# zhizdev/sparsefusion

Measured on AMD Instinct MI355X. Metric: novel views/sec, distillation steps (2 NGP renders fwd+bwd + VAE enc/dec + 51-eval PLMS + LPIPS), 256^2 / 32x32 latents, 2-view synthetic hydrant, higher is better.
Workload: dtype bf16 MFMA operands / f32 accumulate (UNet); f32 (NGP render)

## Files before the change

### include/sparsefusion_hip.h

```cpp
#ifndef SPARSEFUSION_HIP_H
#define SPARSEFUSION_HIP_H

#include <stdint.h>

#ifdef __cplusplus
extern "C" {
#endif

#define SF_OK 0
#define SF_ERR_INVALID 1
#define SF_ERR_LAUNCH 2

const char* sf_last_error(void);
int sf_abi_version(void);
int sf_operand_is_f16(void);


int sf_grid_encode_forward(const float* inputs, const float* embeddings,
                           const int32_t* offsets, float* outputs,
                           uint32_t B, uint32_t D, uint32_t C, uint32_t L,
                           float S, uint32_t H, float* dy_dx,
                           uint32_t gridtype, int align_corners,
                           const int32_t* h_offsets, void* stream);

// ... 82 lines not shown
  float* g_w2; float* g_b2;
} sf_ngp_field_grad;

int sf_ngp_density(const sf_ngp_field* f, const float* xyz, uint32_t P,
                   float* sigma, float* albedo, void* stream);


int sf_ngp_density_lattice(const sf_ngp_field* f, const float* ax, const float* ay, const float* az,
                           uint32_t nx, uint32_t ny, uint32_t nz, float* sigma, void* stream);

int sf_ngp_point_attrs(const sf_ngp_field* f, const float* xyz, uint32_t P, float epsilon,
                       float* sigma, float* albedo, float* grad, float* normal, void* stream);

int sf_ngp_texture_bake(const sf_ngp_field* f, const float* verts, uint32_t V, const int32_t* faces, uint32_t F, uint32_t W,
                        uint8_t* rgb8, float* albedo, float* xyz, int32_t* face_id, void* stream);

uint64_t sf_gaussian3d_workspace_bytes(uint32_t nx, uint32_t ny, uint32_t nz);
int sf_gaussian3d(const float* in, float* out, uint32_t nx, uint32_t ny, uint32_t nz,
                  float sigma, float truncate, double* stats, void* workspace,
                  uint64_t workspace_bytes, void* stream);

uint64_t sf_mc_workspace_bytes(uint32_t nx, uint32_t ny, uint32_t nz);
int sf_mc_count(const float* vol, uint32_t nx, uint32_t ny, uint32_t nz, float iso,
                void* workspace, uint64_t workspace_bytes, uint32_t* counts2, void* stream);
int sf_mc_emit(const float* vol, uint32_t nx, uint32_t ny, uint32_t nz, float iso,
               void* workspace, uint64_t workspace_bytes, float* verts, int32_t* faces,
               void* stream);

int sf_ngp_render_forward(const sf_ngp_field* f, const float* rays_o,
                          const float* rays_d, const float* aabb, uint32_t N,
                          uint32_t T, float min_near, const float* lin,
                          const float* u_coarse, const float* u_fine,
                          uint32_t u_fine_row_stride, float bg_color, float* nears,
                          float* fars, float* z_sorted, float* sigma_s,
                          float* rgb_s, float* image, float* depth,
                          float* weights_sum, float* field_cache, float* workspace,
                          uint64_t workspace_bytes, void* stream);

int sf_ngp_render_backward(const sf_ngp_field* f, const sf_ngp_field_grad* g,
                           const float* rays_o, const float* rays_d,
                           const float* aabb, uint32_t N, uint32_t T,
                           const float* nears, const float* fars,
                           const float* z_sorted, const float* sigma_s,
                           const float* rgb_s, float bg_color,
                           const float* grad_image, const float* grad_weights_sum,
                           uint32_t rays_per_row, const float* field_cache,
                           float* workspace, uint64_t workspace_bytes,
                           void* stream);

uint64_t sf_ngp_render_workspace_bytes(uint32_t N, uint32_t T);
uint64_t sf_ngp_render_forward_workspace_bytes(uint32_t N, uint32_t T);

uint64_t sf_ngp_render_cache_bytes(uint32_t N, uint32_t T);

int sf_ngp_render_shaded_forward(const sf_ngp_field* f, const float* rays_o, const float* rays_d, const float* aabb,
                                 uint32_t N, uint32_t T, float min_near, const float* lin, const float* u_coarse,
                                 const float* u_fine, uint32_t u_fine_row_stride, float bg_color, const float* light_d,
                                 float ambient_ratio, float epsilon, float* nears, float* fars, float* z_sorted,
                                 float* sigma_s, float* rgb_s, float* normal_s, float* rgb_shaded_s, float* xyz_s,
                                 float* image, float* normal_image, float* orient, float* depth, float* weights_sum,
                                 float* workspace, uint64_t workspace_bytes, void* stream);
uint64_t sf_ngp_render_shaded_workspace_bytes(uint32_t N, uint32_t T);

int sf_ngp_render_occ_eval(const sf_ngp_field* f, const float* rays_o, const float* rays_d,
                           const float* nears, const float* fars, const uint8_t* grid,
                           float dt_gamma, uint32_t max_steps, uint32_t C, uint32_t H,
                           const float* noises, float T_thresh, uint32_t N,
                           float* weights_sum, float* depth, float* image, void* stream);

int sf_ngp_render_occ_eval_shaded(const sf_ngp_field* f, const float* rays_o, const float* rays_d,
        const float* nears, const float* fars, const uint8_t* grid, float dt_gamma, uint32_t max_steps,
        uint32_t C, uint32_t H, const float* noises, float T_thresh, uint32_t N,
        const float* light_d , float ambient_ratio, float epsilon,
        float* weights_sum, float* depth, float* image,
        float* normal_image , uint32_t* n_samples ,
        void* stream);


enum {
  SF_OP_CONV = 1,
  SF_OP_GN_ACT = 2,
  SF_OP_LN = 3,
  SF_OP_GEMV = 4,
  SF_OP_ATTN = 5,
  SF_OP_GCA_POOL = 6,
  SF_OP_ELTWISE = 7,
  SF_OP_MEMSET = 8,
  SF_OP_TIME_EMB = 9,
  SF_OP_SPLITK_REDUCE = 10,
  SF_OP_POOL = 11,
  SF_OP_LPIPS = 12,
  SF_OP_EFT = 13,
  SF_OP_FCONV = 14,
  SF_OP_SLOTS = 15,
  SF_OP_GCA = 16,
  SF_OP_INITX = 17,
  SF_OP_GN_FINALIZE = 18
};

typedef struct {
  int32_t type;
  int32_t flags;
  void* p[24];
  int32_t i[32];
  float f[8];
} sf_op;
// ... 61 lines not shown
```

### sparsefusion_amd/_lib.py

```python
import ctypes as C
import os

import torch

_HERE = os.path.dirname(os.path.abspath(__file__))
_DEFAULT_LIB = "libsparsefusion_hip_f16.so" if os.environ.get("SF_OPERAND", "bf16").lower() in ("f16", "fp16", "half") else "libsparsefusion_hip.so"
LIB_PATH = os.environ.get("SF_HIP_LIB") or os.path.join(_HERE, _DEFAULT_LIB)

_lib = None

c_f32p = C.c_void_p
c_i32p = C.c_void_p
u32 = C.c_uint32
u64 = C.c_uint64


class SfNgpField(C.Structure):
    _fields_ = [("embeddings", C.c_void_p), ("h_offsets", C.c_void_p), ("L", u32), ("S", C.c_float),
                ("H", u32), ("gridtype", u32),
                ("w0", C.c_void_p), ("b0", C.c_void_p), ("w1", C.c_void_p), ("b1", C.c_void_p),
                ("w2", C.c_void_p), ("b2", C.c_void_p), ("bound", C.c_float)]


class SfNgpFieldGrad(C.Structure):
# ... 24 lines not shown
    "sf_last_error": (C.c_char_p, []),
    "sf_abi_version": (C.c_int, []),
    "sf_operand_is_f16": (C.c_int, []),
    "sf_grid_encode_forward": (C.c_int, [c_f32p, c_f32p, c_i32p, c_f32p, u32, u32, u32, u32, C.c_float, u32,
                                         c_f32p, u32, C.c_int, C.c_void_p, C.c_void_p]),
    "sf_grid_encode_backward": (C.c_int, [c_f32p, c_f32p, c_f32p, c_i32p, c_f32p, u32, u32, u32, u32, C.c_float,
                                          u32, c_f32p, c_f32p, u32, C.c_int, C.c_void_p, C.c_void_p]),
    "sf_near_far_from_aabb": (C.c_int, [c_f32p, c_f32p, c_f32p, u32, C.c_float, c_f32p, c_f32p, C.c_void_p]),
    "sf_morton3D": (C.c_int, [c_i32p, u32, c_i32p, C.c_void_p]),
    "sf_morton3D_invert": (C.c_int, [c_i32p, u32, c_i32p, C.c_void_p]),
    "sf_packbits": (C.c_int, [c_f32p, u32, C.c_float, C.c_void_p, C.c_void_p]),
    "sf_occ_mark_untrained": (C.c_int, [c_f32p, c_f32p, u32, C.c_float, u32, u32, c_f32p, c_i32p, C.c_void_p, C.c_void_p]),
    "sf_sph_from_ray": (C.c_int, [c_f32p, c_f32p, C.c_float, u32, c_f32p, C.c_void_p]),
    "sf_march_rays_train_workspace_bytes": (u64, [u32]),
    "sf_march_rays_train": (C.c_int, [c_f32p, c_f32p, C.c_void_p, C.c_float, C.c_float, u32, u32, u32, u32, u32, c_f32p,
                                      c_f32p, c_f32p, c_f32p, c_f32p, c_i32p, c_i32p, c_f32p, C.c_void_p, u64, C.c_void_p]),
    "sf_composite_rays_train_forward": (C.c_int, [c_f32p, c_f32p, c_f32p, c_i32p, u32, u32, C.c_float, c_f32p, c_f32p,
                                                  c_f32p, C.c_void_p]),
    "sf_composite_rays_train_backward": (C.c_int, [c_f32p, c_f32p, c_f32p, c_f32p, c_f32p, c_i32p, c_f32p, c_f32p, u32,
                                                   u32, C.c_float, c_f32p, c_f32p, C.c_void_p]),
    "sf_march_rays": (C.c_int, [u32, u32, c_i32p, c_f32p, c_f32p, c_f32p, C.c_float, C.c_float, u32, u32, u32,
                                C.c_void_p, c_f32p, c_f32p, c_f32p, c_f32p, c_f32p, c_f32p, C.c_void_p]),
    "sf_composite_rays": (C.c_int, [u32, u32, C.c_float, c_i32p, c_f32p, c_f32p, c_f32p, c_f32p, c_f32p, c_f32p,
                                    c_f32p, C.c_void_p]),
    "sf_adam_multi": (C.c_int, [C.POINTER(SfAdamArgs), C.c_void_p]),
    "sf_loss_partial_rows": (u32, []),
    "sf_upsample2x_forward": (C.c_int, [c_f32p, c_f32p, u32, u32, u32, C.c_void_p]),
    "sf_upsample2x_backward": (C.c_int, [c_f32p, c_f32p, u32, u32, u32, C.c_void_p]),
    "sf_render_loss_forward": (C.c_int, [c_f32p, c_f32p, c_f32p, c_f32p, u64, u64, C.c_float, c_f32p, C.c_void_p]),
    "sf_render_loss_backward": (C.c_int, [c_f32p, c_f32p, c_f32p, c_f32p, u64, u64, C.c_float, C.c_float, C.c_float, C.c_float,
                                          C.c_float, c_f32p, c_f32p, c_f32p, C.c_void_p]),
    "sf_fusion_loss_forward": (C.c_int, [c_f32p, c_f32p, c_f32p, c_f32p, u32, u64, u64, c_f32p, C.c_void_p]),
    "sf_fusion_loss_backward": (C.c_int, [c_f32p, c_f32p, c_f32p, c_f32p, u32, u64, u64, C.c_float, C.c_float, C.c_float,
                                          c_f32p, c_f32p, c_f32p, C.c_void_p]),
    "sf_ngp_density": (C.c_int, [C.POINTER(SfNgpField), c_f32p, u32, c_f32p, c_f32p, C.c_void_p]),
    "sf_ngp_density_lattice": (C.c_int, [C.POINTER(SfNgpField), c_f32p, c_f32p, c_f32p, u32, u32, u32, c_f32p, C.c_void_p]),
    "sf_ngp_point_attrs": (C.c_int, [C.POINTER(SfNgpField), c_f32p, u32, C.c_float, c_f32p, c_f32p, c_f32p, c_f32p, C.c_void_p]),
    "sf_ngp_texture_bake": (C.c_int, [C.POINTER(SfNgpField), c_f32p, u32, c_i32p, u32, u32, C.c_void_p, c_f32p, c_f32p, c_i32p,
                                      C.c_void_p]),
    "sf_gaussian3d_workspace_bytes": (u64, [u32, u32, u32]),
    "sf_gaussian3d": (C.c_int, [c_f32p, c_f32p, u32, u32, u32, C.c_float, C.c_float, C.c_void_p, C.c_void_p, u64, C.c_void_p]),
    "sf_mc_workspace_bytes": (u64, [u32, u32, u32]),
    "sf_mc_count": (C.c_int, [c_f32p, u32, u32, u32, C.c_float, C.c_void_p, u64, C.c_void_p, C.c_void_p]),
    "sf_mc_emit": (C.c_int, [c_f32p, u32, u32, u32, C.c_float, C.c_void_p, u64, c_f32p, c_i32p, C.c_void_p]),
    "sf_ngp_render_forward": (C.c_int, [C.POINTER(SfNgpField), c_f32p, c_f32p, c_f32p, u32, u32, C.c_float,
                                        c_f32p, c_f32p, c_f32p, u32, C.c_float, c_f32p, c_f32p, c_f32p, c_f32p,
                                        c_f32p, c_f32p, c_f32p, c_f32p, c_f32p, c_f32p, u64, C.c_void_p]),
    "sf_ngp_render_backward": (C.c_int, [C.POINTER(SfNgpField), C.POINTER(SfNgpFieldGrad), c_f32p, c_f32p,
                                         c_f32p, u32, u32, c_f32p, c_f32p, c_f32p, c_f32p, c_f32p,
                                         C.c_float, c_f32p, c_f32p, u32, c_f32p, c_f32p, u64, C.c_void_p]),
    "sf_ngp_render_workspace_bytes": (u64, [u32, u32]),
    "sf_ngp_render_forward_workspace_bytes": (u64, [u32, u32]),
    "sf_ngp_render_cache_bytes": (u64, [u32, u32]),
    "sf_ngp_render_shaded_forward": (C.c_int, [C.POINTER(SfNgpField), c_f32p, c_f32p, c_f32p, u32, u32, C.c_float, c_f32p, c_f32p,
                                               c_f32p, u32, C.c_float, c_f32p, C.c_float, C.c_float, c_f32p, c_f32p, c_f32p,
                                               c_f32p, c_f32p, c_f32p, c_f32p, c_f32p, c_f32p, c_f32p, c_f32p, c_f32p, c_f32p,
                                               c_f32p, u64, C.c_void_p]),
    "sf_ngp_render_shaded_workspace_bytes": (u64, [u32, u32]),
    "sf_ngp_render_occ_eval": (C.c_int, [C.POINTER(SfNgpField), c_f32p, c_f32p, c_f32p, c_f32p, C.c_void_p, C.c_float, u32, u32, u32,
                                         c_f32p, C.c_float, u32, c_f32p, c_f32p, c_f32p, C.c_void_p]),
    "sf_ngp_render_occ_eval_shaded": (C.c_int, [C.POINTER(SfNgpField), c_f32p, c_f32p, c_f32p, c_f32p, C.c_void_p, C.c_float, u32, u32,
                                                u32, c_f32p, C.c_float, u32, c_f32p, C.c_float, C.c_float, c_f32p, c_f32p, c_f32p,
                                                c_f32p, C.c_void_p, C.c_void_p]),
    "sf_plan_run": (C.c_int, [C.POINTER(SfOp), u32, C.c_void_p]),
    "sf_conv_igemm_t_launches": (u64, []),
    "sf_gca4_launches": (u64, [C.c_int]),
    "sf_plan_profile": (C.c_int, [C.POINTER(SfOp), u32, C.c_void_p, C.c_void_p]),
    "sf_conv_packed_elems": (u64, [u32, u32, u32, u32]),
    "sf_conv_pack_weights": (C.c_int, [C.c_void_p, u32, u32, u32, u32, u32, C.c_void_p]),
    "sf_plms_update": (C.c_int, [c_f32p, c_f32p, c_f32p, C.c_void_p, u64, c_f32p, c_f32p, C.c_void_p]),
    "sf_plms_combine": (C.c_int, [c_f32p, c_f32p, c_f32p, c_f32p, C.c_void_p, u64, c_f32p, c_f32p, C.c_void_p]),
    "sf_plms_step": (C.c_int, [c_f32p, c_f32p, c_f32p, c_f32p, C.c_void_p, c_f32p, c_f32p, c_f32p, C.c_void_p, u64, c_f32p, c_f32p, c_f32p, u64, C.c_void_p]),
}


_handles = {}


def _load(path):
    if path not in _handles:
        if not os.path.exists(path):
            raise RuntimeError(
                f"{path} is missing: build it with `python -m sparsefusion_amd.build` (`--f16` for the IEEE-half operand build; "
                "there is no CPU fallback for the sparsefusion_amd hot path)")
        handle = C.CDLL(path)
        for name, (res, args) in SIGNATURES.items():
            fn = getattr(handle, name)
            fn.restype = res
            fn.argtypes = args
        _handles[path] = handle
    return _handles[path]


def lib(operand=None):
    global _lib
    if operand is None:
        if _lib is None:
            _lib = _load(LIB_PATH)
        return _lib
    if operand == "f16":
        return _load(os.path.join(_HERE, "libsparsefusion_hip_f16.so"))
    if operand == "bf16":
        return _load(os.path.join(_HERE, "libsparsefusion_hip.so"))
    raise ValueError(f"unknown MFMA operand type {operand!r} (bf16 | f16)")


# ... 23 lines not shown
```

### sparsefusion_amd/csrc/ngp_render.hip

```cpp

#include "sf_common.h"
#include "ngp_device.h"
#include "ngp_field_lds.h"
#include "ngp_bwd_mfma.h"
#include "ngp_composite_wave.h"
#include "ngp_scatter_bin.h"
#include "ngp_shade.h"
#include <stdlib.h>
#include <mutex>

struct GridLevels;
int sf_fill_levels(GridLevels* lv, const int32_t* offsets_dev, const int32_t* h_offsets, uint32_t L, float S,
                   uint32_t H, hipStream_t st);

template <int MODE>
__global__ __launch_bounds__(256) void k_ngp_field(
    FieldPtrs f, NgpLevels lv, const float* __restrict__ rays_o, const float* __restrict__ rays_d,
    const float* __restrict__ aabb, const float* __restrict__ nears, const float* __restrict__ fars,
    const float* __restrict__ lin, const float* __restrict__ u, const float* __restrict__ z_in,
    const float* __restrict__ xyz_in, uint32_t P, uint32_t T, float* __restrict__ z_out,
    float* __restrict__ sigma, float* __restrict__ rgb, float* __restrict__ feat_out = nullptr) {
  __shared__ __attribute__((aligned(16))) float W[NGP_WTOTAL];
  load_weights_lds(W, f);
  __syncthreads();
  float box[6];
  if (MODE != 2) {
#pragma unroll
    for (int i = 0; i < 6; ++i) box[i] = aabb[i];
  }
  for (uint32_t p = blockIdx.x * blockDim.x + threadIdx.x; p < P; p += gridDim.x * blockDim.x) {
    asm volatile("" ::: "memory");
    float x[3];
    if (MODE == 2) {
      x[0] = xyz_in[p * 3 + 0]; x[1] = xyz_in[p * 3 + 1]; x[2] = xyz_in[p * 3 + 2];
    } else {
      const uint32_t n = p / T, k = p - n * T;
      float z;
      if (MODE == 0) {
        z = ngp_coarse_z(nears[n], fars[n], lin[k], u ? u[p] : -1.0f, T);
        z_out[p] = z;
      } else {
        z = z_in[p];
      }
      const float o[3] = {rays_o[n * 3], rays_o[n * 3 + 1], rays_o[n * 3 + 2]};
      const float d[3] = {rays_d[n * 3], rays_d[n * 3 + 1], rays_d[n * 3 + 2]};
      ngp_point(o, d, z, box, x);
    }
    float x01[3];
    const bool inside = ngp_unit(x, f.bound, x01);
    float feat[NGP_FEAT], h1[NGP_HID], h2[NGP_HID], out[NGP_OUT];
    ngp_encode(lv, f.table, x01, inside, feat);
    if (feat_out) {
#pragma unroll
      for (int j = 0; j < NGP_FEAT / 4; ++j)
        *reinterpret_cast<float4*>(feat_out + (size_t)p * NGP_FEAT + 4 * j) = make_float4(feat[4 * j], feat[4 * j + 1], feat[4 * j + 2], feat[4 * j + 3]);
    }
    ngp_mlp_forward(W, feat, h1, h2, out);
    sigma[p] = expf(out[0] + ngp_blob(x));
    rgb[p * 3 + 0] = ngp_sigmoid(out[1]);
    rgb[p * 3 + 1] = ngp_sigmoid(out[2]);
    rgb[p * 3 + 2] = ngp_sigmoid(out[3]);
// ... 190 lines not shown

extern "C" int sf_ngp_density(const sf_ngp_field* f, const float* xyz, uint32_t P, float* sigma, float* albedo,
                              void* stream) {
  hipStream_t st = (hipStream_t)stream;
  NgpLevels lv;
  if (int rc = sf_ngp_make_levels(f, &lv, st)) return rc;
  if (P == 0) return SF_OK;
  k_ngp_field<2><<<sf_grid_cap(sf_div_up(P, 256)), 256, 0, st>>>(field_ptrs(f), lv, nullptr, nullptr, nullptr, nullptr,
                                                                 nullptr, nullptr, nullptr, nullptr, xyz, P, 1, nullptr,
                                                                 sigma, albedo);
  SF_CHECK_LAUNCH("ngp_density");
  return SF_OK;
}

#ifndef NGP_BWD_CHUNKS
#define NGP_BWD_CHUNKS 2u
#endif
struct NgpChunks { uint32_t n, max_rays, start[66]; };
static NgpChunks ngp_bwd_plan(uint32_t N) {
  NgpChunks c{};
  auto equal = [&](uint32_t k) {
    c.n = k; c.max_rays = N / k;
    for (uint32_t i = 0; i <= k; ++i) c.start[i] = i * (N / k);
  };
  auto ok = [&](uint32_t rays, uint32_t k) { return k >= 1 && rays % k == 0 && (rays / k) % 256 == 0 && rays / k >= 2048; };
  for (uint32_t k = (N + 8191) / 8192; k > NGP_BWD_CHUNKS && k <= 64; ++k)
    if (ok(N, k)) { equal(k); return c; }
  uint32_t k = NGP_BWD_CHUNKS;
  while (k > 1 && !ok(N, k)) --k;
  if (N / k > 8192) {
    uint32_t per = 8192;
    if ((N + per - 1) / per > 64) per = (((N + 63) / 64 + 255) / 256) * 256;
    c.n = (N + per - 1) / per; c.max_rays = per;
    for (uint32_t i = 0; i < c.n; ++i) c.start[i] = i * per;
    c.start[c.n] = N;
    return c;
  }
  equal(k);
  return c;
}
#define SB_CURSOR_WORDS (NGP_MAX_LEVELS * SB_MAX_BUCKETS)
#ifndef SB_LEVELS_BUDGET
#define SB_LEVELS_BUDGET 24
#endif
static uint64_t ngp_bin_entries(uint32_t N, uint32_t T) {
  return (uint64_t)ngp_bwd_plan(N).max_rays * 2 * T * 4 * SB_LEVELS_BUDGET + (uint64_t)SB_CURSOR_WORDS * 64;
}
extern "C" uint64_t sf_ngp_render_workspace_bytes(uint32_t N, uint32_t T) {
  return (uint64_t)(8 + 4 * NGP_MAX_LEVELS) * N * T * sizeof(float) + (uint64_t)SB_CURSOR_WORDS * 4 + ngp_bin_entries(N, T) * 16;
}

extern "C" uint64_t sf_ngp_render_forward_workspace_bytes(uint32_t N, uint32_t T) { return (uint64_t)10 * N * T * sizeof(float); }

extern "C" uint64_t sf_ngp_render_cache_bytes(uint32_t N, uint32_t T) {
  return ((uint64_t)2 * N * T * NGP_FEAT + (uint64_t)N * 2 * T) * sizeof(float);
}

extern "C" int sf_ngp_render_forward(const sf_ngp_field* f, const float* rays_o, const float* rays_d,
                                     const float* aabb, uint32_t N, uint32_t T, float min_near,
                                     const float* lin, const float* u_coarse, const float* u_fine,
                                     uint32_t u_fine_row_stride, float bg_color, float* nears, float* fars,
                                     float* z_sorted, float* sigma_s, float* rgb_s, float* image, float* depth,
                                     float* weights_sum, float* field_cache, float* workspace, uint64_t workspace_bytes,
                                     void* stream) {
  hipStream_t st = (hipStream_t)stream;
  if (N == 0) return SF_OK;
  if (T < 4 || T > 64) SF_FAIL(SF_ERR_INVALID, "ngp_render: T must be in [4,64]");
  if (workspace_bytes < sf_ngp_render_forward_workspace_bytes(N, T)) SF_FAIL(SF_ERR_INVALID, "ngp_render: workspace too small");
  if (!lin || !u_fine) SF_FAIL(SF_ERR_INVALID, "ngp_render: lin and u_fine tables are required");
  NgpLevels lv;
  if (int rc = sf_ngp_make_levels(f, &lv, st)) return rc;
  if (int rc = sf_near_far_from_aabb(rays_o, rays_d, aabb, N, min_near, nears, fars, stream)) return rc;
  const uint64_t NT = (uint64_t)N * T;
  float* z_c = workspace;           float* sig_c = z_c + NT;     float* rgb_c = sig_c + NT;
  float* z_f = rgb_c + 3 * NT;      float* sig_f = z_f + NT;     float* rgb_f = sig_f + NT;
  const FieldPtrs fp = field_ptrs(f);
  const uint32_t P = (uint32_t)NT;
  const uint32_t gridp = sf_grid_cap(sf_div_up(P, 256));
  float* feat_c = field_cache;
  float* feat_f = field_cache ? field_cache + NT * NGP_FEAT : nullptr;
  uint32_t* perm = field_cache ? reinterpret_cast<uint32_t*>(field_cache + 2 * NT * NGP_FEAT) : nullptr;
  k_ngp_field<0><<<gridp, 256, 0, st>>>(fp, lv, rays_o, rays_d, aabb, nears, fars, lin, u_coarse, nullptr, nullptr, P, T,
                                        z_c, sig_c, rgb_c, feat_c);
  SF_CHECK_LAUNCH("ngp_field_coarse");
  const uint32_t gridr = sf_div_up(N, 64);
  k_ngp_sample_fine<<<gridr, 64, 2 * T * 64 * sizeof(float), st>>>(z_c, sig_c, u_fine, u_fine_row_stride, nears, fars,
                                                                  N, T, z_f);
  SF_CHECK_LAUNCH("ngp_sample_fine");
  k_ngp_field<1><<<gridp, 256, 0, st>>>(fp, lv, rays_o, rays_d, aabb, nears, fars, nullptr, nullptr, z_f, nullptr, P, T,
                                        nullptr, sig_f, rgb_f, feat_f);
  SF_CHECK_LAUNCH("ngp_field_fine");
  k_ngp_composite_wave<<<sf_div_up(N, 4), 256, 4 * 5 * 2 * T * sizeof(float), st>>>(
      CompositeArgs{z_c, sig_c, rgb_c, z_f, sig_f, rgb_f, nears, fars, N, T, bg_color, z_sorted, sigma_s, rgb_s, image, depth,
                    weights_sum, perm});
  SF_CHECK_LAUNCH("ngp_composite");
  return SF_OK;
}

extern "C" uint64_t sf_ngp_render_shaded_workspace_bytes(uint32_t N, uint32_t T) { return sf_ngp_render_forward_workspace_bytes(N, T); }

extern "C" int sf_ngp_render_shaded_forward(const sf_ngp_field* f, const float* rays_o, const float* rays_d, const float* aabb,
                                            uint32_t N, uint32_t T, float min_near, const float* lin, const float* u_coarse,
                                            const float* u_fine, uint32_t u_fine_row_stride, float bg_color, const float* light_d,
                                            float ambient_ratio, float epsilon, float* nears, float* fars, float* z_sorted,
                                            float* sigma_s, float* rgb_s, float* normal_s, float* rgb_shaded_s, float* xyz_s,
                                            float* image, float* normal_image, float* orient, float* depth, float* weights_sum,
                                            float* workspace, uint64_t workspace_bytes, void* stream) {
  hipStream_t st = (hipStream_t)stream;
  if (!light_d) SF_FAIL(SF_ERR_INVALID, "ngp_render_shaded: null light_d");
  if (!isfinite(epsilon) || !(epsilon > 0.0f)) SF_FAIL(SF_ERR_INVALID, "ngp_render_shaded: epsilon must be finite and > 0");
  if (!isfinite(ambient_ratio)) SF_FAIL(SF_ERR_INVALID, "ngp_render_shaded: ambient_ratio must be finite");
  if (N == 0) return SF_OK;
  if (T < 4 || T > 64) SF_FAIL(SF_ERR_INVALID, "ngp_render_shaded: T must be in [4,64]");
  if ((uint64_t)N * 2 * T >= (1ull << 32)) SF_FAIL(SF_ERR_INVALID, "ngp_render_shaded: N * 2T must be below 2^32");
  if (workspace_bytes < sf_ngp_render_shaded_workspace_bytes(N, T)) SF_FAIL(SF_ERR_INVALID, "ngp_render_shaded: workspace too small");
  if (!lin || !u_fine) SF_FAIL(SF_ERR_INVALID, "ngp_render_shaded: lin and u_fine tables are required");
  if (!f || !rays_o || !rays_d || !aabb || !nears || !fars || !z_sorted || !sigma_s || !rgb_s || !normal_s || !rgb_shaded_s || !image ||
      !depth || !weights_sum || !workspace)
    SF_FAIL(SF_ERR_INVALID, "ngp_render_shaded: null pointer");
  NgpLevels lv;
  if (int rc = sf_ngp_make_levels(f, &lv, st)) return rc;
  if (int rc = sf_ngp_render_forward(f, rays_o, rays_d, aabb, N, T, min_near, lin, u_coarse, u_fine, u_fine_row_stride, bg_color, nears,
                                     fars, z_sorted, sigma_s, rgb_s, image, depth, weights_sum, nullptr, workspace, workspace_bytes, stream))
    return rc;
  const uint32_t P = N * 2 * T;
  ShadeArgs s{};
  s.f = field_ptrs(f); s.lv = lv;
  s.rays_o = rays_o; s.rays_d = rays_d; s.aabb = aabb; s.z_s = z_sorted; s.rgb_s = rgb_s; s.light_d = light_d;
  s.P = P; s.T2 = 2 * T; s.ratio = ambient_ratio; s.eps = epsilon;
  s.normal_s = normal_s; s.rgb_shaded_s = rgb_shaded_s; s.xyz_s = xyz_s;
  k_ngp_shade<<<sf_grid_cap(sf_div_up(P, 256)), 256, 0, st>>>(s);
  SF_CHECK_LAUNCH("ngp_shade");
  k_ngp_composite_sorted_wave<<<sf_div_up(N, 4), 256, 0, st>>>(
      CompositeSortedArgs{z_sorted, sigma_s, rgb_shaded_s, normal_s, rays_d, nears, fars, N, T, bg_color, image, depth, weights_sum,
                          normal_image, orient});
  SF_CHECK_LAUNCH("ngp_composite_sorted");
  return SF_OK;
}

extern "C" int sf_ngp_render_backward(const sf_ngp_field* f, const sf_ngp_field_grad* g, const float* rays_o,
                                      const float* rays_d, const float* aabb, uint32_t N, uint32_t T,
                                      const float* nears, const float* fars, const float* z_sorted,
                                      const float* sigma_s, const float* rgb_s, float bg_color,
// ... 192 lines not shown
```

### sparsefusion_amd/nerf/renderer.py

```python
import argparse
import ctypes as C
import math
import os

import torch
import torch.nn as nn

from .. import _lib
from .utils import safe_normalize


def get_default_torch_ngp_opt():
    opt = argparse.Namespace()
    opt.cuda_ray = False
    opt.max_steps = 256
    opt.num_steps = 64
    opt.upsample_steps = 64
    opt.update_extra_interval = 16
    opt.max_ray_batch = 4096
    opt.albedo_iters = 1000
    opt.bg_radius = 0
    opt.density_thresh = 10
    opt.fp16 = True
    opt.backbone = 'grid'
    opt.w = 128
    opt.h = 128
    opt.hw_scale = 2
    opt.bound = 4
    opt.min_near = 0.1
    opt.dt_gamma = 0
    opt.lambda_entropy = 1e-4
    opt.lambda_opacity = 0
    opt.lambda_orient = 1e-2
    opt.lambda_smooth = 0
    return opt


class _FieldHandle:

    def __init__(self, net):
        enc = net.encoder
        lin = net.sigma_net.net
        self.tensors = [enc.embeddings, lin[0].weight, lin[0].bias, lin[1].weight, lin[1].bias, lin[2].weight,
                        lin[2].bias]
        self.host_offsets = enc.host_offsets
        self.L = enc.num_levels
        self.S = float(math.log2(enc.per_level_scale))
        self.H = int(enc.base_resolution)
        self.gridtype = int(enc.gridtype_id)
        self.bound = float(net.bound)

    def struct(self, tensors):
        f = _lib.SfNgpField()
        f.embeddings = tensors[0].data_ptr()
        f.h_offsets = self.host_offsets.ctypes.data
        f.L, f.S, f.H, f.gridtype = self.L, self.S, self.H, self.gridtype
        f.w0, f.b0, f.w1, f.b1, f.w2, f.b2 = (t.data_ptr() for t in tensors[1:])
        f.bound = self.bound
        return f


_FEAT_CACHE = True


class _RenderFn(torch.autograd.Function):
    @staticmethod
    def forward(ctx, handle, rays_o, rays_d, aabb, T, min_near, lin, u_coarse, u_fine, u_stride, bg, rays_per_row, grad_mode, *params):
        _lib.require_cuda(rays_o, rays_d, aabb, *params)
        params = [p.detach().contiguous() for p in params]
        N = rays_o.shape[0]
        dev = rays_o.device
        f32 = dict(dtype=torch.float32, device=dev)
        nears, fars = torch.empty(N, **f32), torch.empty(N, **f32)
        z_s, sig_s = torch.empty(N, 2 * T, **f32), torch.empty(N, 2 * T, **f32)
        rgb_s = torch.empty(N, 2 * T, 3, **f32)
        image, depth, ws = torch.empty(N, 3, **f32), torch.empty(N, **f32), torch.empty(N, **f32)
        lib = _lib.lib()
        wbytes = lib.sf_ngp_render_forward_workspace_bytes(N, T)
        work = torch.empty(max(1, wbytes // 4), **f32)
        f = handle.struct(params)
        cache = None
        if _FEAT_CACHE and grad_mode and any(ctx.needs_input_grad[13:]):
            cache = torch.empty(lib.sf_ngp_render_cache_bytes(N, T) // 4, **f32)
        rc = lib.sf_ngp_render_forward(C.byref(f), _lib.ptr(rays_o), _lib.ptr(rays_d), _lib.ptr(aabb), N, T,
                                       float(min_near), _lib.ptr(lin), _lib.ptr(u_coarse), _lib.ptr(u_fine),
                                       int(u_stride), float(bg), _lib.ptr(nears), _lib.ptr(fars), _lib.ptr(z_s),
                                       _lib.ptr(sig_s), _lib.ptr(rgb_s), _lib.ptr(image), _lib.ptr(depth), _lib.ptr(ws),
                                       _lib.ptr(cache), _lib.ptr(work), wbytes, _lib.stream_ptr())
        _lib.check(rc, "ngp_render_forward")
        ctx.handle, ctx.T, ctx.bg, ctx.rays_per_row = handle, T, float(bg), int(rays_per_row)
        ctx.has_cache = cache is not None
        ctx.save_for_backward(rays_o, rays_d, aabb, nears, fars, z_s, sig_s, rgb_s, *([cache] if cache is not None else []), *params)
        ctx.mark_non_differentiable(depth, nears, fars)
        return image, ws, depth, nears, fars

    @staticmethod
    def backward(ctx, g_image, g_ws, _gd, _gn, _gf):
        rays_o, rays_d, aabb, nears, fars, z_s, sig_s, rgb_s, *params = ctx.saved_tensors
        cache = params.pop(0) if ctx.has_cache else None
        N, T = rays_o.shape[0], ctx.T
        grads = [torch.zeros_like(p) for p in params]
        g = _lib.SfNgpFieldGrad()
        (g.g_embeddings, g.g_w0, g.g_b0, g.g_w1, g.g_b1, g.g_w2, g.g_b2) = (t.data_ptr() for t in grads)
        f = ctx.handle.struct(params)
        lib = _lib.lib()
        wbytes = lib.sf_ngp_render_workspace_bytes(N, T)
        work = torch.empty(max(1, wbytes // 4), dtype=torch.float32, device=rays_o.device)
        g_image = (g_image if g_image is not None else torch.zeros(N, 3, device=rays_o.device)).contiguous().float()
        g_ws = g_ws.contiguous().float() if g_ws is not None else None
        rc = lib.sf_ngp_render_backward(C.byref(f), C.byref(g), _lib.ptr(rays_o), _lib.ptr(rays_d), _lib.ptr(aabb), N, T,
                                        _lib.ptr(nears), _lib.ptr(fars), _lib.ptr(z_s), _lib.ptr(sig_s), _lib.ptr(rgb_s),
                                        ctx.bg, _lib.ptr(g_image), _lib.ptr(g_ws), int(ctx.rays_per_row), _lib.ptr(cache),
                                        _lib.ptr(work), wbytes, _lib.stream_ptr())
        _lib.check(rc, "ngp_render_backward")
        return (None,) * 13 + tuple(grads)


class NeRFRenderer(nn.Module):
    def __init__(self, opt):
        super().__init__()
        self.opt = opt
        self.bound = opt.bound
        self.cascade = 1 + math.ceil(math.log2(opt.bound))
        self.grid_size = 128
        self.cuda_ray = opt.cuda_ray
        self.min_near = opt.min_near
        self.density_thresh = opt.density_thresh
        self.bg_radius = opt.bg_radius
        if self.bg_radius > 0:
            raise NotImplementedError("bg_radius > 0 is not on the distillation path (distillation.py:512)")
        box = torch.tensor([-opt.bound] * 3 + [opt.bound] * 3, dtype=torch.float32)
        self.register_buffer('aabb_train', box)
        self.register_buffer('aabb_infer', box.clone())
        self._tables = {}
        if self.cuda_ray:
            self.register_buffer('density_grid', torch.zeros([self.cascade, self.grid_size ** 3]))
# ... 126 lines not shown
        prefix = rays_o.shape[:-1]
        o = rays_o.contiguous().view(-1, 3).float()
        d = rays_d.contiguous().view(-1, 3).float()
        N, T, dev = o.shape[0], int(num_steps), o.device
        aabb = self.aabb_train if self.training else self.aabb_infer
        lin, det = self._table(T, dev)
        if shaded and light_d is not None:
            light = light_d.detach().reshape(3).to(device=dev, dtype=torch.float32)
        elif shaded and fixed_light:
            rot_m = torch.tensor([[0.63, .65, -0.43], [-.43, .75, -0.5], [-.65, .13, .75]], device=dev, dtype=torch.float)
            light = safe_normalize(o[0] @ rot_m)
        else:
            light = None
        if light_d is None and not fixed_light and (noise is None or shaded):
            draw = torch.randn(3, device=dev, dtype=torch.float)
            if shaded:
                light = safe_normalize(o[0] + draw)
        if noise is None:
            u_coarse = torch.rand(N, T, device=dev) if perturb else None
            u_fine = torch.rand(N, T, device=dev) if self.training else None
        else:
            u_coarse, u_fine = noise.get("u_coarse"), noise.get("u_fine")
        u_f, stride = (u_fine.contiguous(), T) if u_fine is not None else (det, 0)
        if u_coarse is not None:
            u_coarse = u_coarse.contiguous()
        if bg_color is None:
            bg_color = 1
        if torch.is_tensor(bg_color):
            raise NotImplementedError("per-ray bg_color tensors are not on the distillation path (bg_color=0)")
        if shaded:
            return self._run_shaded(prefix, o, d, aabb, T, lin, u_coarse, u_f, stride, float(bg_color), light.contiguous(),
                                    float(ambient_ratio))
        image, weights_sum, depth, nears, fars = _RenderFn.apply(
            self._field_handle(), o, d, aabb, T, self.min_near, lin, u_coarse, u_f, stride, float(bg_color),
            self._rays_per_row(N, kwargs), torch.is_grad_enabled(), *self._field_params())
        return {'image': image.view(*prefix, 3), 'depth': depth.view(*prefix), 'weights_sum': weights_sum,
                'mask': (nears < fars).view(*prefix)}

    @torch.no_grad()
    def _run_shaded(self, prefix, o, d, aabb, T, lin, u_coarse, u_fine, u_stride, bg, light, ratio, epsilon=1e-2):
        params = [q.detach().contiguous() for q in self._field_params()]
        _lib.require_cuda(o, d, aabb, light, *params)
        N, dev = o.shape[0], o.device
        f32 = dict(dtype=torch.float32, device=dev)
        nears, fars = torch.empty(N, **f32), torch.empty(N, **f32)
        z_s, sig_s = torch.empty(N, 2 * T, **f32), torch.empty(N, 2 * T, **f32)
        rgb_s, nrm_s, col_s = (torch.empty(N, 2 * T, 3, **f32) for _ in range(3))
        image, nimg = torch.empty(N, 3, **f32), torch.empty(N, 3, **f32)
        depth, ws, orient = torch.empty(N, **f32), torch.empty(N, **f32), torch.empty(N, **f32)
        lib = _lib.lib()
        wbytes = lib.sf_ngp_render_shaded_workspace_bytes(N, T)
        work = torch.empty(max(1, wbytes // 4), **f32)
        f = self._field_handle().struct(params)
        rc = lib.sf_ngp_render_shaded_forward(C.byref(f), _lib.ptr(o), _lib.ptr(d), _lib.ptr(aabb), N, T, float(self.min_near),
                                              _lib.ptr(lin), _lib.ptr(u_coarse), _lib.ptr(u_fine), int(u_stride), bg, _lib.ptr(light),
                                              ratio, float(epsilon), _lib.ptr(nears), _lib.ptr(fars), _lib.ptr(z_s), _lib.ptr(sig_s),
                                              _lib.ptr(rgb_s), _lib.ptr(nrm_s), _lib.ptr(col_s), None, _lib.ptr(image), _lib.ptr(nimg),
                                              _lib.ptr(orient), _lib.ptr(depth), _lib.ptr(ws), _lib.ptr(work), wbytes, _lib.stream_ptr())
        _lib.check(rc, "ngp_render_shaded_forward")
        return {'image': image.view(*prefix, 3), 'depth': depth.view(*prefix), 'weights_sum': ws, 'mask': (nears < fars).view(*prefix),
                'loss_orient': orient.sum() / max(1, N * 2 * T), 'normal': nimg.view(*prefix, 3)}

    @staticmethod
    def _rays_per_row(N, kwargs):
        w, h = kwargs.get('w'), kwargs.get('h')
        return int(w) if w and h and int(w) * int(h) == N else 0

    def run_cuda(self, rays_o, rays_d, dt_gamma=0, light_d=None, ambient_ratio=1.0, shading='albedo', bg_color=None,
                 perturb=False, force_all_rays=False, max_steps=1024, T_thresh=1e-4, noise=None, **kwargs):
        from .. import raymarching
        if shading not in ('albedo', 'lambertian'):
            raise NotImplementedError(f"shading={shading!r}: only 'albedo' and 'lambertian' are rendered ('textureless' and 'normal' use "
                                      "the reference's random smooth normal, common_forward_smooth, which is not reproduced)")
        shaded = shading == 'lambertian'
        if shaded and self.training:
            raise NotImplementedError("shading='lambertian' through the occupancy grid is an evaluation render (call .eval() first): "
                                      "the three-stage training path (march_rays_train / field / composite_rays_train) has no shaded "
                                      "form; only shading='albedo' is on the distillation path (distillation.py:209,282)")
        if shaded and light_d is not None:
            light_d = torch.as_tensor(light_d)
            if light_d.numel() != 3:
                raise ValueError("light_d must be a 3-vector")
        lead = rays_o.shape[:-1]
        o = rays_o.contiguous().view(-1, 3).float()
        d = rays_d.contiguous().view(-1, 3).float()
        if shaded:
            _lib.require_cuda(o, d)
        box = self.aabb_train if self.training else self.aabb_infer
        nears, fars = raymarching.near_far_from_aabb(o, d, box)
        if shaded:
            if light_d is not None:
                light = light_d.detach().reshape(3).to(device=o.device, dtype=torch.float32)
            else:
                light = safe_normalize(o[0] + torch.randn(3, device=o.device, dtype=torch.float))
            opacity, z, rgb, nimg = self._occ_eval_shaded(o, d, nears, fars, dt_gamma, perturb, max_steps, T_thresh, noise,
                                                          light.contiguous(), float(ambient_ratio))
            background = 1 if bg_color is None else bg_color
            rgb = rgb + (1 - opacity).unsqueeze(-1) * background
            return {'image': rgb.view(*lead, 3),
                    'depth': (torch.clamp(z - nears, min=0) / (fars - nears)).view(*lead),
                    'weights_sum': opacity.reshape(*lead),
                    'mask': (nears < fars).reshape(*lead),
                    'normal': nimg.view(*lead, 3)}
        stage = self._occ_train if self.training else self._occ_eval
        opacity, z, rgb = stage(o, d, nears, fars, dt_gamma, perturb, force_all_rays, max_steps, T_thresh, noise, ambient_ratio)
        background = 1 if bg_color is None else bg_color
# ... 94 lines not shown
```

Before: 18.08.

## Add MFMA-based NGP field forward kernel with prefetched hash-grid gathers

Adds a new forward kernel for the NGP field that handles 32 points per wave. The hash-grid encoding is split across the two half-waves, and table gathers are prefetched one level ahead. The two hidden MLP layers run on f32 MFMA instructions, with weights staged in LDS and layer-1 weights held in registers. It is enabled by default for both the coarse and fine field passes, with a runtime toggle to fall back to the old scalar kernel. The aim is to replace per-thread scalar FMA MLP evaluation with matrix-core throughput, at the cost of LDS usage, a grid cap and more register pressure.

```diff
diff --git a/include/sparsefusion_hip.h b/include/sparsefusion_hip.h
--- a/include/sparsefusion_hip.h
+++ b/include/sparsefusion_hip.h
@@ -158,6 +158,8 @@
 uint64_t sf_ngp_render_forward_workspace_bytes(uint32_t N, uint32_t T);
 
 uint64_t sf_ngp_render_cache_bytes(uint32_t N, uint32_t T);
+
+int sf_ngp_field_mfma(int on);
 
 int sf_ngp_render_shaded_forward(const sf_ngp_field* f, const float* rays_o, const float* rays_d, const float* aabb,
                                  uint32_t N, uint32_t T, float min_near, const float* lin, const float* u_coarse,
diff --git a/sparsefusion_amd/_lib.py b/sparsefusion_amd/_lib.py
--- a/sparsefusion_amd/_lib.py
+++ b/sparsefusion_amd/_lib.py
@@ -100,6 +100,7 @@
     "sf_ngp_render_workspace_bytes": (u64, [u32, u32]),
     "sf_ngp_render_forward_workspace_bytes": (u64, [u32, u32]),
     "sf_ngp_render_cache_bytes": (u64, [u32, u32]),
+    "sf_ngp_field_mfma": (C.c_int, [C.c_int]),
     "sf_ngp_render_shaded_forward": (C.c_int, [C.POINTER(SfNgpField), c_f32p, c_f32p, c_f32p, u32, u32, C.c_float, c_f32p, c_f32p,
                                                c_f32p, u32, C.c_float, c_f32p, C.c_float, C.c_float, c_f32p, c_f32p, c_f32p,
                                                c_f32p, c_f32p, c_f32p, c_f32p, c_f32p, c_f32p, c_f32p, c_f32p, c_f32p, c_f32p,
diff --git a/sparsefusion_amd/csrc/ngp_field_mfma.h b/sparsefusion_amd/csrc/ngp_field_mfma.h
--- /dev/null
+++ b/sparsefusion_amd/csrc/ngp_field_mfma.h
@@ -0,0 +1,220 @@
+#pragma once
+#include "sf_dev.h"
+#include "ngp_device.h"
+
+#define FM_PTS 32
+#define FM_SF 33
+#define FM_SH 65
+#define FM_WAVE_FLOATS (FM_PTS * FM_SF + FM_PTS * FM_SH)
+#define FM_W2 0
+#define FM_B2 (FM_W2 + NGP_OUT * NGP_HID)
+#define FM_B0 (FM_B2 + 8)
+#define FM_B1 (FM_B0 + NGP_HID)
+#define FM_W0 (FM_B1 + NGP_HID)
+#define FM_HEAD (FM_W0 + NGP_HID * FM_SF)
+#define FM_LDS_FLOATS (FM_HEAD + 4 * FM_WAVE_FLOATS)
+
+#ifndef FM_DEPTH
+#define FM_DEPTH 1
+#endif
+
+#ifdef SF_HOST_EMU
+#define FM_SCHED_FENCE() do { } while (0)
+#else
+#define FM_SCHED_FENCE() __builtin_amdgcn_sched_barrier(0)
+#endif
+
+struct FMArgs {
+  const float* table; const float* w0; const float* b0; const float* w1; const float* b1; const float* w2; const float* b2;
+  float bound;
+  NgpLevels lv;
+  const float* rays_o; const float* rays_d; const float* aabb; const float* nears; const float* fars;
+  const float* lin; const float* u;
+  const float* z_in;
+  uint32_t P, T;
+  float* z_out;
+  float* sigma; float* rgb;
+  float* feat_out;
+};
+
+SF_DEV void fm_level(const NgpLevels& lv, uint32_t hi, int ll, NgpLevels& m) {
+  m.scale[0] = hi ? lv.scale[8 + ll] : lv.scale[ll];
+  m.resolution[0] = hi ? lv.resolution[8 + ll] : lv.resolution[ll];
+  m.offset[0] = hi ? lv.offset[8 + ll] : lv.offset[ll];
+  m.hsize[0] = hi ? lv.hsize[8 + ll] : lv.hsize[ll];
+  m.gridtype = lv.gridtype;
+}
+
+template <int MODE>
+SF_KERNEL(256) void k_ngp_field_mfma(FMArgs a) {
+  SF_DYN_LDS(lds_raw);
+  float* W = reinterpret_cast<float*>(lds_raw);
+  const int tid = threadIdx.x, lane = tid & 63, wave = tid >> 6;
+  const int li = lane & 15, kq = lane >> 4;
+  float bw1[NGP_HID / 4][4];
+  {
+    float* S1 = W + FM_HEAD;
+    for (int i = tid; i < NGP_HID * NGP_FEAT; i += 256) W[FM_W0 + (i >> 5) * FM_SF + (i & 31)] = a.w0[i];
+    for (int i = tid; i < NGP_HID * NGP_HID; i += 256) S1[(i >> 6) * FM_SH + (i & 63)] = a.w1[i];
+    for (int i = tid; i < NGP_OUT * NGP_HID; i += 256) W[FM_W2 + i] = a.w2[i];
+    if (tid < NGP_HID) { W[FM_B0 + tid] = a.b0[tid]; W[FM_B1 + tid] = a.b1[tid]; }
+    if (tid < NGP_OUT) W[FM_B2 + tid] = a.b2[tid];
+    sf_sync();
+#pragma unroll
+    for (int nt = 0; nt < 4; ++nt) {
+#pragma unroll
+      for (int s = 0; s < NGP_HID / 4; ++s) bw1[s][nt] = S1[(nt * 16 + li) * FM_SH + 4 * s + kq];
+    }
+    sf_sync();
+  }
+  float* F = W + FM_HEAD + wave * FM_WAVE_FLOATS;
+  float* H = F + FM_PTS * FM_SF;
+  float box[6];
+#pragma unroll
+  for (int i = 0; i < 6; ++i) box[i] = a.aabb[i];
+
+  const int pl = lane & 31, half = lane >> 5;
+  const uint32_t n_trips = (a.P + FM_PTS - 1) / FM_PTS;
+  for (uint32_t trip = blockIdx.x * 4 + wave; trip < n_trips; trip += gridDim.x * 4) {
+    const uint32_t p = trip * FM_PTS + pl;
+    const bool live = p < a.P;
+    float x01[3] = {0.f, 0.f, 0.f}, blob = 0.0f;
+    bool inside = false;
+    if (live) {
+      const uint32_t n = p / a.T;
+      float z;
+      if (MODE == 0) {
+        z = ngp_coarse_z(a.nears[n], a.fars[n], a.lin[p - n * a.T], a.u ? a.u[p] : -1.0f, a.T);
+        if (half == 0) a.z_out[p] = z;
+      } else {
+        z = a.z_in[p];
+      }
+      const float o[3] = {a.rays_o[n * 3], a.rays_o[n * 3 + 1], a.rays_o[n * 3 + 2]};
+      const float d[3] = {a.rays_d[n * 3], a.rays_d[n * 3 + 1], a.rays_d[n * 3 + 2]};
+      float x[3];
+      ngp_point(o, d, z, box, x);
+      inside = ngp_unit(x, a.bound, x01);
+      blob = ngp_blob(x);
+    }
+    const float xe[3] = {inside ? x01[0] : 0.0f, inside ? x01[1] : 0.0f, inside ? x01[2] : 0.0f};
+    uint32_t hi = half;
+    SF_USE_FROM_HERE(hi);
+    f32x2 fv[FM_DEPTH][8];
+    float w[FM_DEPTH][8];
+    NgpCell c;
+    NgpLevels m;
+#pragma unroll
+    for (int q = 0; q < FM_DEPTH; ++q) {
+      fm_level(a.lv, hi, q, m);
+      ngp_cell(m, 0, xe, c);
+      const float* tab = a.table + (size_t)m.offset[0] * 2;
+#pragma unroll
+      for (int i = 0; i < 8; ++i) {
+        fv[q][i] = *reinterpret_cast<const f32x2*>(tab + (size_t)c.row[i] * 2);
+        w[q][i] = c.w[i];
+      }
+      FM_SCHED_FENCE();
+    }
+#pragma unroll
+    for (int ll = 0; ll < 8; ++ll) {
+      const uint32_t l = hi * 8 + ll;
+      const int q = ll % FM_DEPTH;
+      const float* tab = a.table;
+      if (ll + FM_DEPTH < 8) {
+        fm_level(a.lv, hi, ll + FM_DEPTH, m);
+        ngp_cell(m, 0, xe, c);
+        tab = a.table + (size_t)m.offset[0] * 2;
+      }
+      FM_SCHED_FENCE();
+      float r0 = 0.0f, r1 = 0.0f;
+#pragma unroll
+      for (int i = 0; i < 8; ++i) {
+        r0 = fmaf(w[q][i], fv[q][i][0], r0);
+        r1 = fmaf(w[q][i], fv[q][i][1], r1);
+      }
+      if (!(inside && l < a.lv.L)) r0 = r1 = 0.0f;
+      F[pl * FM_SF + 2 * l] = r0;
+      F[pl * FM_SF + 2 * l + 1] = r1;
+      if (ll + FM_DEPTH < 8) {
+#pragma unroll
+        for (int i = 0; i < 8; ++i) {
+          fv[q][i] = *reinterpret_cast<const f32x2*>(tab + (size_t)c.row[i] * 2);
+          w[q][i] = c.w[i];
+        }
+      }
+      FM_SCHED_FENCE();
+    }
+    if (a.feat_out && live) {
+      float* dst = a.feat_out + (size_t)p * NGP_FEAT + half * 16;
+#pragma unroll
+      for (int j = 0; j < 4; ++j) {
+        f32x4 v;
+#pragma unroll
+        for (int e = 0; e < 4; ++e) v[e] = F[pl * FM_SF + half * 16 + 4 * j + e];
+        *reinterpret_cast<f32x4*>(dst + 4 * j) = v;
+      }
+    }
+    sf_wave_sync();
+
+#pragma unroll
+    for (int mt = 0; mt < 2; ++mt) {
+      f32x4 c[4];
+#pragma unroll
+      for (int nt = 0; nt < 4; ++nt) {
+        const float bv = W[FM_B0 + nt * 16 + li];
+        c[nt] = f32x4{bv, bv, bv, bv};
+      }
+#pragma unroll
+      for (int s = 0; s < NGP_FEAT / 4; ++s) {
+        const float av = F[(mt * 16 + li) * FM_SF + 4 * s + kq];
+#pragma unroll
+        for (int nt = 0; nt < 4; ++nt) c[nt] = sf_mfma4(av, W[FM_W0 + (nt * 16 + li) * FM_SF + 4 * s + kq], c[nt]);
+      }
+#pragma unroll
+      for (int nt = 0; nt < 4; ++nt)
+#pragma unroll
+        for (int r = 0; r < 4; ++r) H[(mt * 16 + 4 * kq + r) * FM_SH + nt * 16 + li] = fmaxf(c[nt][r], 0.0f);
+    }
+    sf_wave_sync();
+#pragma unroll
+    for (int mt = 0; mt < 2; ++mt) {
+      f32x4 c[4];
+#pragma unroll
+      for (int nt = 0; nt < 4; ++nt) {
+        const float bv = W[FM_B1 + nt * 16 + li];
+        c[nt] = f32x4{bv, bv, bv, bv};
+      }
+#pragma unroll
+      for (int s = 0; s < NGP_HID / 4; ++s) {
+        const float av = H[(mt * 16 + li) * FM_SH + 4 * s + kq];
+#pragma unroll
+        for (int nt = 0; nt < 4; ++nt) c[nt] = sf_mfma4(av, bw1[s][nt], c[nt]);
+      }
+      sf_wave_sync();
+#pragma unroll
+      for (int nt = 0; nt < 4; ++nt)
+#pragma unroll
+        for (int r = 0; r < 4; ++r) H[(mt * 16 + 4 * kq + r) * FM_SH + nt * 16 + li] = fmaxf(c[nt][r], 0.0f);
+    }
+    sf_wave_sync();
+    {
+      float o0 = W[FM_B2 + 2 * half], o1 = W[FM_B2 + 2 * half + 1];
+#pragma unroll 8
+      for (int k = 0; k < NGP_HID; ++k) {
+        const float hk = H[pl * FM_SH + k];
+        o0 = fmaf(W[FM_W2 + (2 * half) * NGP_HID + k], hk, o0);
+        o1 = fmaf(W[FM_W2 + (2 * half + 1) * NGP_HID + k], hk, o1);
+      }
+      if (live) {
+        if (half == 0) {
+          a.sigma[p] = expf(o0 + blob);
+          a.rgb[(size_t)p * 3 + 0] = ngp_sigmoid(o1);
+        } else {
+          a.rgb[(size_t)p * 3 + 1] = ngp_sigmoid(o0);
+          a.rgb[(size_t)p * 3 + 2] = ngp_sigmoid(o1);
+        }
+      }
+    }
+    sf_wave_sync();
+  }
+}
diff --git a/sparsefusion_amd/csrc/ngp_render.hip b/sparsefusion_amd/csrc/ngp_render.hip
--- a/sparsefusion_amd/csrc/ngp_render.hip
+++ b/sparsefusion_amd/csrc/ngp_render.hip
@@ -3,10 +3,12 @@
 #include "ngp_device.h"
 #include "ngp_field_lds.h"
 #include "ngp_bwd_mfma.h"
+#include "ngp_field_mfma.h"
 #include "ngp_composite_wave.h"
 #include "ngp_scatter_bin.h"
 #include "ngp_shade.h"
 #include <stdlib.h>
+#include <atomic>
 #include <mutex>
 
 struct GridLevels;
@@ -303,6 +305,16 @@
 
 extern "C" uint64_t sf_ngp_render_forward_workspace_bytes(uint32_t N, uint32_t T) { return (uint64_t)10 * N * T * sizeof(float); }
 
+#ifndef FM_GRID_CAP
+#define FM_GRID_CAP 512u
+#endif
+static std::atomic<int> g_field_mfma{1};
+extern "C" int sf_ngp_field_mfma(int on) {
+  const int was = g_field_mfma.load(std::memory_order_relaxed);
+  if (on >= 0) g_field_mfma.store(on ? 1 : 0, std::memory_order_relaxed);
+  return was;
+}
+
 extern "C" uint64_t sf_ngp_render_cache_bytes(uint32_t N, uint32_t T) {
   return ((uint64_t)2 * N * T * NGP_FEAT + (uint64_t)N * 2 * T) * sizeof(float);
 }
@@ -331,15 +343,31 @@
   float* feat_c = field_cache;
   float* feat_f = field_cache ? field_cache + NT * NGP_FEAT : nullptr;
   uint32_t* perm = field_cache ? reinterpret_cast<uint32_t*>(field_cache + 2 * NT * NGP_FEAT) : nullptr;
-  k_ngp_field<0><<<gridp, 256, 0, st>>>(fp, lv, rays_o, rays_d, aabb, nears, fars, lin, u_coarse, nullptr, nullptr, P, T,
-                                        z_c, sig_c, rgb_c, feat_c);
+  const bool mfma = g_field_mfma.load(std::memory_order_relaxed) != 0;
+  FMArgs fm{};
+  fm.table = fp.table; fm.w0 = fp.w0; fm.b0 = fp.b0; fm.w1 = fp.w1; fm.b1 = fp.b1; fm.w2 = fp.w2; fm.b2 = fp.b2; fm.bound = fp.bound;
+  fm.lv = lv; fm.rays_o = rays_o; fm.rays_d = rays_d; fm.aabb = aabb; fm.nears = nears; fm.fars = fars; fm.P = P; fm.T = T;
+  const uint32_t gridm = sf_div_up(sf_div_up(P, FM_PTS), 4) < FM_GRID_CAP ? sf_div_up(sf_div_up(P, FM_PTS), 4) : FM_GRID_CAP;
+  const size_t ldsm = FM_LDS_FLOATS * sizeof(float);
+  if (mfma) {
+    fm.lin = lin; fm.u = u_coarse; fm.z_out = z_c; fm.sigma = sig_c; fm.rgb = rgb_c; fm.feat_out = feat_c;
+    k_ngp_field_mfma<0><<<gridm, 256, ldsm, st>>>(fm);
+  } else {
+    k_ngp_field<0><<<gridp, 256, 0, st>>>(fp, lv, rays_o, rays_d, aabb, nears, fars, lin, u_coarse, nullptr, nullptr, P, T,
+                                          z_c, sig_c, rgb_c, feat_c);
+  }
   SF_CHECK_LAUNCH("ngp_field_coarse");
   const uint32_t gridr = sf_div_up(N, 64);
   k_ngp_sample_fine<<<gridr, 64, 2 * T * 64 * sizeof(float), st>>>(z_c, sig_c, u_fine, u_fine_row_stride, nears, fars,
                                                                   N, T, z_f);
   SF_CHECK_LAUNCH("ngp_sample_fine");
-  k_ngp_field<1><<<gridp, 256, 0, st>>>(fp, lv, rays_o, rays_d, aabb, nears, fars, nullptr, nullptr, z_f, nullptr, P, T,
-                                        nullptr, sig_f, rgb_f, feat_f);
+  if (mfma) {
+    fm.lin = nullptr; fm.u = nullptr; fm.z_in = z_f; fm.z_out = nullptr; fm.sigma = sig_f; fm.rgb = rgb_f; fm.feat_out = feat_f;
+    k_ngp_field_mfma<1><<<gridm, 256, ldsm, st>>>(fm);
+  } else {
+    k_ngp_field<1><<<gridp, 256, 0, st>>>(fp, lv, rays_o, rays_d, aabb, nears, fars, nullptr, nullptr, z_f, nullptr, P, T,
+                                          nullptr, sig_f, rgb_f, feat_f);
+  }
   SF_CHECK_LAUNCH("ngp_field_fine");
   k_ngp_composite_wave<<<sf_div_up(N, 4), 256, 4 * 5 * 2 * T * sizeof(float), st>>>(
       CompositeArgs{z_c, sig_c, rgb_c, z_f, sig_f, rgb_f, nears, fars, N, T, bg_color, z_sorted, sigma_s, rgb_s, image, depth,
diff --git a/sparsefusion_amd/nerf/renderer.py b/sparsefusion_amd/nerf/renderer.py
--- a/sparsefusion_amd/nerf/renderer.py
+++ b/sparsefusion_amd/nerf/renderer.py
@@ -61,6 +61,11 @@
 
 
 _FEAT_CACHE = True
+_FIELD_MFMA = True
+
+
+def _select_field_kernel(lib):
+    lib.sf_ngp_field_mfma(1 if _FIELD_MFMA else 0)
 
 
 class _RenderFn(torch.autograd.Function):
@@ -82,6 +87,7 @@
         cache = None
         if _FEAT_CACHE and grad_mode and any(ctx.needs_input_grad[13:]):
             cache = torch.empty(lib.sf_ngp_render_cache_bytes(N, T) // 4, **f32)
+        _select_field_kernel(lib)
         rc = lib.sf_ngp_render_forward(C.byref(f), _lib.ptr(rays_o), _lib.ptr(rays_d), _lib.ptr(aabb), N, T,
                                        float(min_near), _lib.ptr(lin), _lib.ptr(u_coarse), _lib.ptr(u_fine),
                                        int(u_stride), float(bg), _lib.ptr(nears), _lib.ptr(fars), _lib.ptr(z_s),
@@ -314,6 +320,7 @@
         wbytes = lib.sf_ngp_render_shaded_workspace_bytes(N, T)
         work = torch.empty(max(1, wbytes // 4), **f32)
         f = self._field_handle().struct(params)
+        _select_field_kernel(lib)
         rc = lib.sf_ngp_render_shaded_forward(C.byref(f), _lib.ptr(o), _lib.ptr(d), _lib.ptr(aabb), N, T, float(self.min_near),
                                               _lib.ptr(lin), _lib.ptr(u_coarse), _lib.ptr(u_fine), int(u_stride), bg, _lib.ptr(light),
                                               ratio, float(epsilon), _lib.ptr(nears), _lib.ptr(fars), _lib.ptr(z_s), _lib.ptr(sig_s),
```

Result: faster. 18.28 (median of 6 runs) (+1.1%).
